# GAMES-UChile/mogptk

Hardware: AMD Instinct MI355X
Metric: log-marginal-likelihood+grad evals/sec, MOSM C=4 N=8192; 1/2/4/8 GPU (higher is better)
Workload: dtype f64

## Files before the change

include/mogp_hip.h:

```cpp
#ifndef MOGP_HIP_H
#define MOGP_HIP_H

#include <stdint.h>

#ifdef __cplusplus
extern "C" {
#endif

#define MOGP_OK            0
#define MOGP_EINVAL       -1
#define MOGP_EHIP         -2
#define MOGP_ENOTPD       -3
#define MOGP_ENONFINITE   -4
#define MOGP_ENODEVICE    -5

#define MOGP_TERM_WIDTH(D) (2 + 3 * (D))
#define MOGP_MOMENT_WIDTH(D) (2 + 3 * (D))

typedef struct mogp_ctx mogp_ctx;
typedef struct mogp_model mogp_model;

const char* mogp_version(void);
const char* mogp_last_error(void);
int  mogp_device_count(void);
// ... 91 lines not shown
int  mogp_stage_ms(mogp_model* m, double* ms, int64_t* gemm_launches, double* gemm_flops);

#define MOGP_SCHED_DATAFLOW            1
#define MOGP_SCHED_CHAIN_KERNEL        2
#define MOGP_SCHED_DATAFLOW_FELL_BACK  4
#define MOGP_SCHED_TIMEOUTS_SHIFT      8
#define MOGP_SCHED_CHAIN_FELL_BACK     8
int  mogp_model_schedule(mogp_model* m, int* flags);

int  mogp_model_flow_replay(mogp_model* m, int on);

int  mogp_model_flow_diag(mogp_model* m, unsigned* out8);

int  mogp_flow_plan(int nb, int64_t* out, int64_t cap, int64_t* count);
int  mogp_flow_plan_rhs(int nb, int rhs_nt, int64_t* out, int64_t cap, int64_t* count);
int  mogp_flow_trace(mogp_model* m, int64_t* out, int64_t cap, int64_t* count);

int  mogp_model_fetch(mogp_model* m, int which, double* out);

int  mogp_snelson_eval(mogp_model* m, int64_t M, const double* Z, const double* noise_var, double jitter, const double* kff_diag, int flags,
                       double* lml, double* mom_uu, double* mom_uf, double* gZ, double* trGA, double* hsum, double* jitter_abs, int64_t* info);
int  mogp_snelson_predict(mogp_model* m, int64_t M, const double* Z, const double* noise_var, double jitter, const double* kff_diag,
                          const double* kss_diag, int64_t S, const double* Xs, double* mu, double* var, int64_t* info);
int  mogp_snelson_eval_sharded(mogp_model* m, int64_t M, const double* Z, const double* noise_var, double jitter, const double* kff_diag,
                               int flags, double* lml, double* mom_uu, double* mom_uf, double* gZ, double* trGA, double* hsum,
                               double* jitter_abs, int64_t* info);
int  mogp_snelson_predict_sharded(mogp_model* m, int64_t M, const double* Z, const double* noise_var, double jitter, const double* kff_diag,
                                  const double* kss_diag, int64_t S, const double* Xs, double* mu, double* var, int64_t* info);

int  mogp_svgp_forward(mogp_model* m, int64_t M, const double* Z, const double* q_mu, const double* q_sqrt, double jitter,
// ... 25 lines not shown
```

mogptk_amd/_lib.py:

```python
import atexit
import ctypes
import os
import threading
import weakref
import numpy as np

_HERE = os.path.dirname(os.path.abspath(__file__))
LIB_PATH = os.environ.get("MOGP_LIB_PATH") or os.path.join(_HERE, "csrc", "libmogp_hip.so")

MOGP_OK, MOGP_EINVAL, MOGP_EHIP, MOGP_ENOTPD, MOGP_ENONFINITE, MOGP_ENODEVICE = 0, -1, -2, -3, -4, -5
MOGP_EVAL_GRAD = 1
COMM_ID_BYTES = 128
ALLGATHER_CB = ctypes.CFUNCTYPE(ctypes.c_int, ctypes.c_void_p, ctypes.c_void_p, ctypes.c_void_p, ctypes.c_int64)
ALLREDUCE_CB = ctypes.CFUNCTYPE(ctypes.c_int, ctypes.c_void_p, ctypes.c_void_p, ctypes.c_int64)
ST_GRAM, ST_POTRF, ST_TRTRI, ST_LAUUM, ST_SOLVE, ST_MOMENTS, ST_TOTAL, ST_GEMM_KERNEL, ST_GRAM_KERNEL, ST_MOMENT_KERNEL, ST_COUNT = range(11)

_lib = None
_lock = threading.RLock()
_ctx = {}
_live = weakref.WeakSet()

c_dp = ctypes.POINTER(ctypes.c_double)
c_i64p = ctypes.POINTER(ctypes.c_int64)
c_ip = ctypes.POINTER(ctypes.c_int)
# ... 56 lines not shown
    "mogp_shard_begin": (ctypes.c_int, [ctypes.c_void_p, c_dp, c_dp, ctypes.c_double, c_dp, ctypes.POINTER(ctypes.c_int)]),
    "mogp_shard_pack": (ctypes.c_int, [ctypes.c_void_p, ctypes.c_int, ctypes.POINTER(ctypes.c_void_p), ctypes.POINTER(ctypes.c_void_p), c_i64p]),
    "mogp_shard_unpack": (ctypes.c_int, [ctypes.c_void_p, ctypes.c_int]),
    "mogp_shard_block": (ctypes.c_int, [ctypes.c_void_p, ctypes.c_int]),
    "mogp_shard_alpha": (ctypes.c_int, [ctypes.c_void_p, ctypes.POINTER(ctypes.c_void_p), c_i64p]),
    "mogp_shard_finish": (ctypes.c_int, [ctypes.c_void_p, c_dp, c_dp, c_dp, c_i64p]),
    "mogp_dev_copy": (ctypes.c_int, [ctypes.c_void_p, ctypes.c_void_p, ctypes.c_int64, ctypes.c_int]),
    "mogp_set_profiling": (ctypes.c_int, [ctypes.c_void_p, ctypes.c_int]),
    "mogp_stage_ms": (ctypes.c_int, [ctypes.c_void_p, c_dp, c_i64p, c_dp]),
    "mogp_model_fetch": (ctypes.c_int, [ctypes.c_void_p, ctypes.c_int, c_dp]),
    "mogp_model_schedule": (ctypes.c_int, [ctypes.c_void_p, ctypes.POINTER(ctypes.c_int)]),
    "mogp_model_flow_replay": (ctypes.c_int, [ctypes.c_void_p, ctypes.c_int]),
    "mogp_model_flow_diag": (ctypes.c_int, [ctypes.c_void_p, ctypes.POINTER(ctypes.c_uint)]),
    "mogp_flow_plan": (ctypes.c_int, [ctypes.c_int, c_i64p, ctypes.c_int64, c_i64p]),
    "mogp_flow_plan_rhs": (ctypes.c_int, [ctypes.c_int, ctypes.c_int, c_i64p, ctypes.c_int64, ctypes.POINTER(ctypes.c_int64)]),
    "mogp_flow_trace": (ctypes.c_int, [ctypes.c_void_p, c_i64p, ctypes.c_int64, c_i64p]),
    "mogp_snelson_eval": (ctypes.c_int, [ctypes.c_void_p, ctypes.c_int64, c_dp, c_dp, ctypes.c_double, c_dp, ctypes.c_int,
                                         ctypes.POINTER(ctypes.c_double), c_dp, c_dp, c_dp, ctypes.POINTER(ctypes.c_double), c_dp,
                                         ctypes.POINTER(ctypes.c_double), c_i64p]),
    "mogp_snelson_predict": (ctypes.c_int, [ctypes.c_void_p, ctypes.c_int64, c_dp, c_dp, ctypes.c_double, c_dp, c_dp, ctypes.c_int64, c_dp,
                                            c_dp, c_dp, c_i64p]),
    "mogp_snelson_eval_sharded": (ctypes.c_int, [ctypes.c_void_p, ctypes.c_int64, c_dp, c_dp, ctypes.c_double, c_dp, ctypes.c_int,
                                         ctypes.POINTER(ctypes.c_double), c_dp, c_dp, c_dp, ctypes.POINTER(ctypes.c_double), c_dp,
                                         ctypes.POINTER(ctypes.c_double), c_i64p]),
    "mogp_snelson_predict_sharded": (ctypes.c_int, [ctypes.c_void_p, ctypes.c_int64, c_dp, c_dp, ctypes.c_double, c_dp, c_dp, ctypes.c_int64, c_dp,
                                            c_dp, c_dp, c_i64p]),
    "mogp_svgp_forward": (ctypes.c_int, [ctypes.c_void_p, ctypes.c_int64, c_dp, c_dp, c_dp, ctypes.c_double, c_dp, ctypes.c_int, ctypes.c_int64,
                                         c_dp, c_dp, c_dp, c_dp, ctypes.POINTER(ctypes.c_double), c_i64p]),
    "mogp_svgp_backward": (ctypes.c_int, [ctypes.c_void_p, c_dp, c_dp, c_dp, c_dp, c_dp, ctypes.POINTER(ctypes.c_double), c_dp, c_dp]),
    "mogp_svgp_backward_sharded": (ctypes.c_int, [ctypes.c_void_p, c_dp, c_dp, c_dp, c_dp, c_dp, ctypes.POINTER(ctypes.c_double), c_dp, c_dp]),
# ... 477 lines not shown
```

mogptk_amd/csrc/flow.hip:

```cpp
#include "mogp_model.h"
#include <unistd.h>
#include <chrono>
#include <set>

#include <cstdio>
#include <cstdlib>

namespace mogp {

typedef double d4_t __attribute__((ext_vector_type(4)));
typedef double d2_t __attribute__((ext_vector_type(2)));

#define FL_BK 16
#define FL_ROWK 18
#define FL_WTM 4
#define FL_WTN 2
#define FL_NWJ 4
#define FL_NWI 2
#define FL_NT 512
#define FL_COLK (MOGP_TILE + 16)
#define FL_OPER (MOGP_TILE * FL_ROWK)
#define FL_LDS_DOUBLES (2 * 2 * FL_OPER)
#define FL_LDS_BYTES (FL_LDS_DOUBLES * 8 + 16 + 3 * 64 * 4 + 16)
static_assert(MOGP_TILE * FL_ROWK == 16 * FL_COLK, "one LDS operand slot serves both layouts");

#define FL_LDS_BARRIER() asm volatile("s_waitcnt lgkmcnt(0)\n\ts_barrier" ::: "memory")

template <int AKM, int BKM, bool MARK = false>
__device__ __forceinline__ void flow_tile(const double* Ap, const double* Bp, double* Cp, const int64_t ld, const int kt, const bool fresh,
                                          const double alpha, double* gemm_lds, unsigned long long* tr, unsigned* prog, double* const* Cpp, const double* alphap) {
    constexpr int WTM = FL_WTM, WTN = FL_WTN, NWJ = FL_NWJ, NWI = FL_NWI, NT = FL_NT;
    constexpr int TMR = MOGP_TILE, TNC = MOGP_TILE, COLK_A = FL_COLK, COLK_B = FL_COLK, OPER_A = FL_OPER, OPER_B = FL_OPER;
    constexpr int EPT_A = TMR * FL_BK / NT, EPT_B = TNC * FL_BK / NT;
    constexpr int NQ_A = EPT_A / 2, NQ_B = EPT_B / 2, TPR_A = FL_BK / EPT_A, TPR_B = FL_BK / EPT_B, TPK = NT / FL_BK;
    int tl = threadIdx.x;
    asm volatile("" : "+v"(tl));
    const int ln = tl & 63, wv = tl >> 6, wi = wv / NWJ, wj = wv % NWJ;
    const int64_t a_g = AKM ? (int64_t)(tl / TPK) * ld + (tl % TPK) * EPT_A : (int64_t)(tl / TPR_A) * ld + (tl % TPR_A) * EPT_A;
    const int64_t b_g = BKM ? (int64_t)(tl / TPK) * ld + (tl % TPK) * EPT_B : (int64_t)(tl / TPR_B) * ld + (tl % TPR_B) * EPT_B;
    const int a_l = AKM ? (tl / TPK) * COLK_A + (tl % TPK) * EPT_A : (tl / TPR_A) * FL_ROWK + (tl % TPR_A) * EPT_A;
    const int b_l = BKM ? (tl / TPK) * COLK_B + (tl % TPK) * EPT_B : (tl / TPR_B) * FL_ROWK + (tl % TPR_B) * EPT_B;
    const int64_t a_step = AKM ? (int64_t)FL_BK * ld : FL_BK;
    const int64_t b_step = BKM ? (int64_t)FL_BK * ld : FL_BK;
    const int crow = wi * (TMR / NWI) + (ln >> 4), ccol = wj * (TNC / NWJ) + (ln & 15);
    const int fa = AKM ? (ln >> 4) * COLK_A + wi * (TMR / NWI) + (ln & 15) : (wi * (TMR / NWI) + (ln & 15)) * FL_ROWK + (ln >> 4);
    const int fb = BKM ? (ln >> 4) * COLK_B + wj * (TNC / NWJ) + (ln & 15) : (wj * (TNC / NWJ) + (ln & 15)) * FL_ROWK + (ln >> 4);
    constexpr int fa_m = AKM ? 16 : 16 * FL_ROWK, fa_k = AKM ? 4 * COLK_A : 4;
    constexpr int fb_n = BKM ? 16 : 16 * FL_ROWK, fb_k = BKM ? 4 * COLK_B : 4;

    d4_t acc[WTM][WTN];
    if (!fresh) {
#pragma unroll
        for (int m = 0; m < WTM; ++m)
#pragma unroll
            for (int n = 0; n < WTN; ++n)
#pragma unroll
                for (int r = 0; r < 4; ++r) acc[m][n][r] = alpha * Cp[(int64_t)(crow + m * 16 + 4 * r) * ld + ccol + n * 16];
    } else {
#pragma unroll
        for (int m = 0; m < WTM; ++m)
#pragma unroll
            for (int n = 0; n < WTN; ++n) acc[m][n] = (d4_t){0.0, 0.0, 0.0, 0.0};
    }
    d2_t ra[NQ_A], rb[NQ_B];
    auto load_block = [&](int kb) {
        const d2_t* pa = reinterpret_cast<const d2_t*>(Ap + a_g + (int64_t)kb * a_step);
        const d2_t* pb = reinterpret_cast<const d2_t*>(Bp + b_g + (int64_t)kb * b_step);
#pragma unroll
        for (int q = 0; q < NQ_A; ++q) ra[q] = pa[q];
#pragma unroll
        for (int q = 0; q < NQ_B; ++q) rb[q] = pb[q];
    };
// ... 1 lines not shown
        double* sa = gemm_lds + buf * (OPER_A + OPER_B);
        double* sb = sa + OPER_A;
#pragma unroll
        for (int q = 0; q < NQ_A; ++q) *reinterpret_cast<d2_t*>(sa + a_l + 2 * q) = ra[q];
#pragma unroll
        for (int q = 0; q < NQ_B; ++q) *reinterpret_cast<d2_t*>(sb + b_l + 2 * q) = rb[q];
    };
    auto read_frag = [&](double (&av)[WTM], double (&bv)[WTN], int buf, int k4) {
        const double* sa = gemm_lds + buf * (OPER_A + OPER_B);
        const double* sb = sa + OPER_A;
#pragma unroll
        for (int m = 0; m < WTM; ++m) av[m] = sa[fa + m * fa_m + k4 * fa_k];
#pragma unroll
        for (int n = 0; n < WTN; ++n) bv[n] = sb[fb + n * fb_n + k4 * fb_k];
    };
    auto mma = [&](const double (&av)[WTM], const double (&bv)[WTN]) {
#pragma unroll
        for (int m = 0; m < WTM; ++m)
#pragma unroll
            for (int n = 0; n < WTN; ++n)
                acc[m][n] = __builtin_amdgcn_mfma_f64_16x16x4f64(av[m], bv[n], acc[m][n], 0, 0, 0);
    };
#define FL_MARK(v) do { if constexpr (MARK) { if (prog && ln == 0) { const unsigned v__ = (v); prog[wv] = v__; \
        if (wv == 0) { const unsigned kb__ = v__ & 0xffffu, now__ = (unsigned)(wall_clock64() >> 4); \
            if (v__ == 0x10000u) prog[8] = now__; else if (v__ == 0x30000u) prog[13] = now__; else if (v__ == 0x40000u) prog[14] = now__; \
            else if ((v__ >> 16) == 2u && (kb__ & 7u) == 0u) prog[9 + (kb__ >> 3)] = now__; } } } } while (0)
    FL_MARK(0x10000u);
    load_block(0);
    write_block(0);
    load_block(min(1, kt - 1));
    FL_LDS_BARRIER();
    if constexpr (MARK) { if (tr) tr[2] = wall_clock64(); }
    {
        double a0[WTM], b0[WTN], a1[WTM], b1[WTN];
        read_frag(a0, b0, 0, 0);
        for (int kb = 0; kb < kt; ++kb) {
            const int buf = kb & 1;
            read_frag(a1, b1, buf, 1);
            __builtin_amdgcn_sched_barrier(0);
            mma(a0, b0);
            __builtin_amdgcn_sched_barrier(0);
            read_frag(a0, b0, buf, 2);
            __builtin_amdgcn_sched_barrier(0);
            mma(a1, b1);
            __builtin_amdgcn_sched_barrier(0);
            write_block(buf ^ 1);
            FL_MARK(0x20000u + (unsigned)kb);
            load_block(min(kb + 2, kt - 1));
            read_frag(a1, b1, buf, 3);
            __builtin_amdgcn_sched_barrier(0);
            mma(a0, b0);
            __builtin_amdgcn_sched_barrier(0);
            FL_LDS_BARRIER();
            read_frag(a0, b0, buf ^ 1, 0);
            __builtin_amdgcn_sched_barrier(0);
            mma(a1, b1);
            __builtin_amdgcn_sched_barrier(0);
        }
    }
    FL_MARK(0x30000u);
    if constexpr (MARK) { if (tr) tr[3] = wall_clock64(); }
    int t2 = threadIdx.x;
    asm volatile("" : "+v"(t2));
    const int ln2 = t2 & 63, wv2 = t2 >> 6;
    const int crow2 = (wv2 / NWJ) * (TMR / NWI) + (ln2 >> 4), ccol2 = (wv2 % NWJ) * (TNC / NWJ) + (ln2 & 15);
    double* Cq = *Cpp;
    const double alpha2 = *alphap;
#pragma unroll
    for (int m = 0; m < WTM; ++m)
#pragma unroll
        for (int n = 0; n < WTN; ++n)
#pragma unroll
            for (int r = 0; r < 4; ++r)
                __hip_atomic_store(Cq + (int64_t)(crow2 + m * 16 + 4 * r) * ld + ccol2 + n * 16, alpha2 * acc[m][n][r], __ATOMIC_RELAXED,
                                   __HIP_MEMORY_SCOPE_AGENT);
    FL_MARK(0x40000u);
#undef FL_MARK
}

struct FlowArgs {
    double* bA; double* bL; double* bWt; double* bWm; double* bB;
    int64_t ld;
    const FlowTask* tasks;
    const int* qmeta;
    unsigned* flags;
    int nq, ncas, base_heads, base_err;
    unsigned nap_max;
    unsigned nap_calm;
    int nhi;
    int claim_one;
    int refill;
    const double* vy; double* vz; double* vzz; double* vpart;
    int64_t npad;
    unsigned long long* info;
    int post_base;
    unsigned char* done;
    unsigned* post;
    unsigned* diag;
    unsigned long long* trace;
};

struct FlowHot {
    double* bA; double* bL; double* bWt; double* bWm; double* bB; int64_t ld;
    const FlowTask* tasks; const int* qmeta; unsigned* flags;
    int nq, ncas, base_heads, base_err;
    unsigned nap_max, nap_calm;
};

__device__ __forceinline__ void flow_zrow(const FlowArgs& g, const int i, double* lds) {
    int tid = threadIdx.x;
    asm volatile("" : "+v"(tid));
    const int lane = tid & 63, wave = tid >> 6;
    const int K = (i + 1) * MOGP_TILE;
    const double* Wr = g.bWm + (int64_t)(i * MOGP_TILE + wave * 16) * g.ld + 2 * lane;
    const double* yp = g.vy + 2 * lane;
    double zsq = 0.0;
    for (int r4 = 0; r4 < 16; r4 += 4) {
        const double* p0 = Wr + (int64_t)r4 * g.ld;
        d2_t a0 = (d2_t){0.0, 0.0}, a1 = a0, a2 = a0, a3 = a0;
#pragma unroll 2
        for (int k = 0; k < K; k += MOGP_TILE) {
// ... 213 lines not shown
                if (lane == 0) { po[0] = (unsigned)(res + 4); po[1] = idle; po[2] = 3u; po[5] = (unsigned)(wall_clock64() >> 4); }
            }
        }
        __syncthreads();
        const int ti = __builtin_amdgcn_readfirstlane(pick[0]);
        if (ti < 0) {
            if (ti == -3 && tid == 0) atomicMin(g.info, (unsigned long long)MOGP_INFO_CHAIN_TIMEOUT);
            break;
        }
        const FlowTask* tp = ha.tasks + ti;
        const int var = tp->var, kt = tp->kt;
        const int ab = tp->abuf, bb = tp->bbuf, cb = tp->cbuf;
        const double* Ab = ab == 0 ? ha.bA : ab == 1 ? ha.bL : ab == 2 ? ha.bWt : ab == 3 ? ha.bWm : ha.bB;
        const double* Bb = bb == 0 ? ha.bA : bb == 1 ? ha.bL : bb == 2 ? ha.bWt : bb == 3 ? ha.bWm : ha.bB;
        double* Cb = cb == 0 ? ha.bA : cb == 1 ? ha.bL : cb == 2 ? ha.bWt : cb == 3 ? ha.bWm : ha.bB;
        const double* Ap = Ab + ((int64_t)tp->ar * ha.ld + tp->ac) * MOGP_TILE;
        const double* Bp = Bb + ((int64_t)tp->br * ha.ld + tp->bc) * MOGP_TILE;
        double* Cp = Cb + ((int64_t)tp->cr * ha.ld + tp->cc) * MOGP_TILE;
        const bool fresh = (var & 4) != 0;
        const double alpha = (var & 8) ? -1.0 : 1.0;
        unsigned long long* tr = (MARK && g.trace && tid == 0) ? g.trace + FLOW_TRACE_W * (size_t)ti : nullptr;
        if (tr) { tr[0] = t_look; tr[1] = wall_clock64(); }
        unsigned* prog = (MARK && g.post) ? g.post + (size_t)(g.post_base + blockIdx.x) * FLOW_POST_W + 80 : nullptr;
        if (MARK && g.post && tid == 0) {
            unsigned* po = g.post + (size_t)(g.post_base + blockIdx.x) * FLOW_POST_W;
            po[2] = 2u; po[3] = (unsigned)ti; po[73] += 1u; po[76] = (unsigned)(wall_clock64() >> 4);
        }
        if (var & 32) {
            if (g.vy) {
                if (var & 1) flow_apart(g, tp->ar * MOGP_TILE, kt * MOGP_TILE, tp->br, tp->ac, gemm_lds);
                else flow_zrow(g, tp->ar, gemm_lds);
            }
        } else {
        if (var & 16) __builtin_amdgcn_s_setprio(2);
        if (tid == 0) { *ep_C = Cp; *ep_alpha = alpha; }
        switch (var & 3) {
            case 0: flow_tile<0, 0, MARK>(Ap, Bp, Cp, ha.ld, kt, fresh, alpha, gemm_lds, tr, prog, ep_C, ep_alpha); break;
            case 1: flow_tile<0, 1, MARK>(Ap, Bp, Cp, ha.ld, kt, fresh, alpha, gemm_lds, tr, prog, ep_C, ep_alpha); break;
            default: flow_tile<1, 1, MARK>(Ap, Bp, Cp, ha.ld, kt, fresh, alpha, gemm_lds, tr, prog, ep_C, ep_alpha); break;
        }
        if (var & 16) __builtin_amdgcn_s_setprio(0);
        }
        asm volatile("s_waitcnt vmcnt(0)" ::: "memory");
        __syncthreads();
        if (tid == 0) {
            const unsigned s0 = tp->sig[0], s1 = tp->sig[1];
            if (s0 != FLOW_NOSIG) __hip_atomic_fetch_add(ha.flags + s0, 1u, __ATOMIC_RELAXED, __HIP_MEMORY_SCOPE_AGENT);
            if (s1 != FLOW_NOSIG) __hip_atomic_fetch_add(ha.flags + s1, 1u, __ATOMIC_RELAXED, __HIP_MEMORY_SCOPE_AGENT);
            if (MARK && g.done) g.done[ti] = 1;
            if (MARK && g.post) g.post[(size_t)(g.post_base + blockIdx.x) * FLOW_POST_W + 77] = (unsigned)(wall_clock64() >> 4);
            if (tr) {
                tr[4] = wall_clock64();
                tr[5] = ((unsigned long long)(unsigned)pick[1] << 32) | ((unsigned long long)__builtin_amdgcn_s_getreg((3 << 11) | 20) << 16) | blockIdx.x;
            }
        }
    }
}


namespace {
enum { PH_INTO = 0, PH_CHAIN = 600, PH_T6 = 601, PH_PANEL = 602, PH_UPDATE = 603, PH_T9 = 604, PH_ZROW = 605, PH_APART = 606, PH_XS = 607, PH_TU = 608 };
enum { Q_LOOK2 = 0, Q_INVCRIT = 1, Q_SEMI = 2 };
enum { BUF_A = 0, BUF_L = 1, BUF_WT = 2, BUF_WM = 3, BUF_B = 4 };
}

void flow_build(int nb, int ob, FlowPlan& p, int rhs_nt, bool replay) {
    p = FlowPlan();
    p.nb = nb; p.ob = ob; p.rhs_nt = rhs_nt; p.replay = replay;
    const int no = (nb + ob - 1) / ob;
    p.nouter = no;
    const uint32_t base_S = 0, base_R = base_S + (uint32_t)nb * nb, base_DG = base_R + (uint32_t)nb * no, base_PN = base_DG + no,
                   base_CH = base_PN + (uint32_t)no * nb, base_WT = base_CH + no, base_WC = base_WT + (uint32_t)nb * nb,
                   base_WF = base_WC + (uint32_t)no * nb, base_KV = base_WF + (uint32_t)no * nb, base_WR = base_KV + (uint32_t)nb * nb,
                   base_ZR = base_WR + no, base_TS = base_ZR + no, base_TR = base_TS + (uint32_t)rhs_nt * nb, base_XN = base_TR + (uint32_t)rhs_nt * no,
                   base_end = base_XN + (uint32_t)no * rhs_nt;
    p.base_heads = (int)base_end; p.base_err = p.base_heads + FLOW_MAXQ; p.nflags = p.base_err + 1;
    auto S = [&](int i, int j) { return base_S + (uint32_t)i * nb + j; };
    auto R = [&](int i, int c) { return base_R + (uint32_t)i * no + c; };
// ... 19 lines not shown
    std::vector<std::vector<FlowTask>> into(no), trail(no);
    auto mk = [&](int b, int phase, int var, int kt) {
        FlowTask t{};
        t.var = (uint8_t)var; t.kt = (uint16_t)kt; t.ndep = 0; t.sig[0] = t.sig[1] = FLOW_NOSIG; t.key = (uint32_t)(b * FLOW_KEY_STEP + phase);
        return t;
    };
    auto dep = [&](FlowTask& t, uint32_t idx, unsigned need) {
        if (need == 0) return;
        t.dep[t.ndep] = idx; t.need[t.ndep] = (uint16_t)need; ++t.ndep;
    };
    auto opA = [](FlowTask& t, int buf, int r, int c) { t.abuf = (uint8_t)buf; t.ar = (uint16_t)r; t.ac = (uint16_t)c; };
    auto opB = [](FlowTask& t, int buf, int r, int c) { t.bbuf = (uint8_t)buf; t.br = (uint16_t)r; t.bc = (uint16_t)c; };
    auto opC = [](FlowTask& t, int buf, int r, int c) { t.cbuf = (uint8_t)buf; t.cr = (uint16_t)r; t.cc = (uint16_t)c; };
    const int KB = MOGP_TILE / FL_BK;
    double tiles_k = 0.0;

    auto crit_row = [&](int b, int i) { return !replay && i >= k1(b) && i < std::min(nb, k1(b) + ob); };
    auto pn_need = [&](int b, int i) { return (unsigned)((crit_row(b, i) ? 2 : 1) * nk(b)); };
    auto panel = [&](int b, int i, int c, bool prio) {
        FlowTask t = mk(b, PH_PANEL, 0 | 4 | (prio ? 16 : 0), KB * (c + 1));
        opA(t, BUF_A, i, k0(b)); opB(t, BUF_WM, k0(b) + c, k0(b)); opC(t, BUF_L, i, k0(b) + c);
        dep(t, CH(b), chain_wgs(b));
        dep(t, R(i, b), (unsigned)(nk(b) * b));
        t.sig[0] = PN(b, i);
        tiles_k += t.kt;
        return t;
    };
    auto update = [&](int b, int i, int j, bool prio) {
        FlowTask t = mk(b, PH_UPDATE, 0 | 8 | (prio ? 16 : 0), KB * nk(b));
        opA(t, BUF_L, i, k0(b)); opB(t, BUF_L, j, k0(b)); opC(t, BUF_A, i, j);
        dep(t, PN(b, i), pn_need(b, i));
        if (j != i) dep(t, PN(b, j), pn_need(b, j));
        dep(t, S(i, j), (unsigned)b);
        t.sig[0] = S(i, j);
        t.sig[1] = blk(i) == blk(j) ? DG(blk(j)) : R(i, blk(j));
        tiles_k += t.kt;
        return t;
    };
    auto t7 = [&](int b, int i, int c) {
        FlowTask t = mk(blk(i), PH_INTO + 2 * b, 1 | 4 | 8, KB * (nk(b) - c));
        opA(t, BUF_L, i, k0(b) + c); opB(t, BUF_WM, k0(b) + c, k0(b) + c); opC(t, BUF_WT, i, k0(b) + c);
        dep(t, PN(b, i), pn_need(b, i));
        t.sig[0] = WT(i, k0(b) + c); t.sig[1] = WC(blk(i), k0(b) + c);
        tiles_k += t.kt;
        return t;
    };
    auto t8 = [&](int b, int i, int j) {
        FlowTask t = mk(blk(i), PH_INTO + 2 * b + 1, 1 | 8, KB * nk(b));
        opA(t, BUF_L, i, k0(b)); opB(t, BUF_WM, k0(b), j); opC(t, BUF_WT, i, j);
        dep(t, PN(b, i), pn_need(b, i));
        dep(t, WF(b, j), (unsigned)nk(b));
        dep(t, WT(i, j), (unsigned)(b - blk(j)));
        t.sig[0] = WT(i, j); t.sig[1] = WC(blk(i), j);
        tiles_k += t.kt;
        return t;
    };
    auto t6 = [&](int b, int ti, int j) {
        FlowTask t = mk(b, PH_T6, 1 | 4, KB * (ti + 1));
        opA(t, BUF_WM, k0(b) + ti, k0(b)); opB(t, BUF_WT, k0(b), j); opC(t, BUF_WM, k0(b) + ti, j);
        dep(t, CH(b), chain_wgs(b));
        dep(t, WC(b, j), (unsigned)(nk(b) * (b - blk(j))));
        t.sig[0] = WF(b, j); t.sig[1] = WR(b);
        tiles_k += t.kt;
        return t;
    };
    static const bool t9_full = std::getenv("MOGP_FLOW_T9FULL") && std::atoi(std::getenv("MOGP_FLOW_T9FULL")) != 0;
    auto t9 = [&](int b, int i, int j) {
        const int r0 = (i >= k0(b) && !t9_full) ? i : k0(b);
        FlowTask t = mk(b, PH_T9, 2 | (i >= k0(b) ? 4 : 0), KB * (k1(b) - r0));
        opA(t, BUF_WM, r0, i); opB(t, BUF_WM, r0, j); opC(t, BUF_B, i, j);
        bool ch = false;
        if (i >= k0(b)) { dep(t, CH(b), chain_wgs(b)); ch = true; } else dep(t, WF(b, i), (unsigned)nk(b));
        if (j != i) { if (j >= k0(b)) { if (!ch) dep(t, CH(b), chain_wgs(b)); } else dep(t, WF(b, j), (unsigned)nk(b)); }
        dep(t, KV(i, j), (unsigned)(b - blk(i)));
        t.sig[0] = KV(i, j);
        tiles_k += t.kt;
        return t;
    };

    auto xs = [&](int b, int i, int c) {
        FlowTask t = mk(b, PH_XS, 0 | 4, KB * (c + 1));
        opA(t, BUF_WT, i, k0(b)); opB(t, BUF_WM, k0(b) + c, k0(b)); opC(t, BUF_B, i, k0(b) + c);
        dep(t, CH(b), chain_wgs(b));
        dep(t, TR(i, b), (unsigned)(nk(b) * b));
        t.sig[0] = XN(b, i);
        tiles_k += t.kt;
        return t;
    };
    auto tu = [&](int b, int i, int j) {
        FlowTask t = mk(b, PH_TU, 0 | 8, KB * nk(b));
        opA(t, BUF_B, i, k0(b)); opB(t, BUF_L, j, k0(b)); opC(t, BUF_WT, i, j);
        dep(t, XN(b, i), (unsigned)nk(b));
        dep(t, PN(b, j), pn_need(b, j));
        dep(t, TS(i, j), (unsigned)b);
        t.sig[0] = TS(i, j); t.sig[1] = TR(i, blk(j));
        tiles_k += t.kt;
        return t;
    };
    std::vector<FlowTask> rrest;

// ... 56 lines not shown
    if ((int)order.size() > FLOW_MAXQ) {
        std::vector<FlowTask> rest;
        std::vector<const std::vector<FlowTask>*> tail(order.begin() + (FLOW_MAXQ - 2), order.end() - 1);
        for (auto* v : tail) rest.insert(rest.end(), v->begin(), v->end());
        std::stable_sort(rest.begin(), rest.end(), [](const FlowTask& x, const FlowTask& y) { return x.key < y.key; });
        p.folded = rest;
        order.erase(order.begin() + (FLOW_MAXQ - 2), order.end() - 1);
        order.insert(order.end() - 1, &p.folded);
    }
    p.nq = (int)order.size();
    for (int qi = 0; qi < p.nq; ++qi) {
        p.qbase[qi] = (int)p.tasks.size(); p.qsize[qi] = (int)order[qi]->size();
        p.tasks.insert(p.tasks.end(), order[qi]->begin(), order[qi]->end());
    }
    p.flops = 2.0 * MOGP_TILE * MOGP_TILE * FL_BK * tiles_k;
}

__global__ void k_alpha_sum(const double* __restrict__ part, int64_t npad, int no, int ob, double* __restrict__ out) {
    const int64_t col = (int64_t)blockIdx.x * blockDim.x + threadIdx.x;
    if (col >= npad) return;
    double s = 0.0;
    for (int r = (int)(col / MOGP_TILE) / ob; r < no; ++r) s += part[(int64_t)r * npad + col];
    out[col] = s;
}
int launch_flow_alpha_sum(const Spd& w, double* alpha, hipStream_t st) {
    const FlowPlan& p = w.flow_cur ? *w.flow_cur : w.flow;
    hipLaunchKernelGGL(k_alpha_sum, dim3((unsigned)((w.Npad + 255) / 256)), dim3(256), 0, st, w.vec_part, w.Npad, p.nouter, p.ob, alpha);
    HIP_TRY(hipGetLastError());
    return 0;
}

bool flow_enabled(const mogp_model* m, const Spd& w) {
    const char* eo = std::getenv("MOGP_FLOW");
    const char* en = std::getenv("MOGP_FLOW_MIN");
    const int on = eo ? std::atoi(eo) : 1, nmin = en ? std::atoi(en) : 8;
    if (!on || (m->no_flow && m->n_fact < m->flow_retry_at) || !chain_enabled(m) || !m->ctx->st_priv) return false;
    if (m->kinv_sparse && &w == &m->k) return false;
    return w.nb >= nmin && w.nb <= 0xfff0;
}

int spd_potri_flow(mogp_model* m, Spd& w, const FlowRhs* rhs) {
    const int nb = w.nb, ob = 4;
    const int64_t ld = w.Npad;
    int rc;
    const auto host_t0 = std::chrono::steady_clock::now();
    hipStream_t crit = m->st, priv = m->st_priv, bulk = m->st2;
    if (w.Wm.n < (size_t)ld * ld) {
        if ((rc = w.Wm.ensure((size_t)ld * ld))) return rc;
        HIP_TRY(hipMemsetAsync(w.Wm.p, 0, (size_t)ld * ld * sizeof(double), crit));
    }
    if ((rc = w.Lm.ensure((size_t)ld * ld))) return rc;
    if (!rhs && (rc = w.Wt.ensure((size_t)ld * ld))) return rc;
    const bool replay = m->replay_flow && !rhs && &w == &m->k;
    FlowPlan& plan = rhs ? w.flow_rhs : replay ? w.flow_replay : w.flow;
    DevBuf<FlowTask>& d_tasks = rhs ? w.flow_tasks_rhs : replay ? w.flow_tasks_replay : w.flow_tasks;
    DevBuf<int>& d_qmeta = rhs ? w.flow_qmeta_rhs : replay ? w.flow_qmeta_replay : w.flow_qmeta;
    const int rhs_nt = rhs ? rhs->nt : 0;
    if (plan.nb != nb || plan.ob != ob || plan.rhs_nt != rhs_nt) {
        flow_build(nb, ob, plan, rhs_nt, replay);
// ... 89 lines not shown
        char* held = w.flow_args_h.data() + slot;
        char* fresh_ = w.flow_args_h.data() + 1024 + slot;
        std::memset(fresh_, 0, 512);
        std::memcpy(fresh_, &a, sizeof(a));
        if (std::memcmp(held, fresh_, 512) == 0) return 0;
        HIP_TRY(hipStreamSynchronize(st));
        HIP_TRY(dev_upload(w.flow_args.p + slot, fresh_, 512));
        std::memcpy(held, fresh_, 512);
        return 0;
    };
    if ((rc = upload(0, g, bulk))) return rc;
    const FlowArgs* d_g = reinterpret_cast<const FlowArgs*>(w.flow_args.p);
    FlowHot hot{};
    hot.bA = g.bA; hot.bL = g.bL; hot.bWt = g.bWt; hot.bWm = g.bWm; hot.bB = g.bB; hot.ld = g.ld; hot.tasks = g.tasks; hot.qmeta = g.qmeta; hot.flags = g.flags;
    hot.nq = g.nq; hot.ncas = g.ncas; hot.base_heads = g.base_heads; hot.base_err = g.base_err; hot.nap_max = g.nap_max; hot.nap_calm = g.nap_calm;
    if (dbg_kernel) hipLaunchKernelGGL(k_flow<true>, dim3(wg_per_cu * cus), dim3(FL_NT), FL_LDS_BYTES, bulk, d_g, hot);
    else hipLaunchKernelGGL(k_flow<false>, dim3(wg_per_cu * cus), dim3(FL_NT), FL_LDS_BYTES, bulk, d_g, hot);
    HIP_TRY(hipGetLastError());
    if (pe1) HIP_TRY(hipEventRecord(pe1, bulk));
    HIP_TRY(hipEventRecord(e_flow, bulk));
    m->gemm_launches += 1;
    m->gemm_flops += p.flops;

    unsigned* ferr = w.flow_flags.p + p.base_err;
    for (int kb = 0; kb < nouter && !replay; ++kb) {
        const int k0 = kb * ob, k1 = std::min(k0 + ob, nb), nk = k1 - k0, na = std::min(ob, nb - k1);
        const FlowPlan::Chain& pc = p.chain[kb];
        ChainFlow cf{};
        cf.done_flag = w.flow_flags.p + pc.done_idx; cf.write_through = 1;
        cf.trace = want_trace ? w.flow_trace.p + FLOW_TRACE_W * p.tasks.size() + 4 * (size_t)kb : nullptr;
        cf.diag = w.flow_diag.p;
        if ((rc = launch_chain(w.A.p, ld, k0, nk, w.invd.p, w.logdet.p, m->d_info.p, 0, w.Wm.p + (int64_t)k0 * MOGP_TILE * (ld + 1), ld,
                               w.chain_flags.p + (size_t)kb * MOGP_CHAIN_FLAGS, ferr, priv, &cf))) return rc;
        if (na <= 0) continue;
        GemmArgs t1{};
        t1.A = w.A.p + (int64_t)k1 * MOGP_TILE * ld + (int64_t)k0 * MOGP_TILE; t1.lda = ld; t1.a_kmajor = 0;
        t1.B = w.Wm.p + (int64_t)k0 * MOGP_TILE * (ld + 1); t1.ldb = ld; t1.b_kmajor = 0;
// ... 245 lines not shown
        std::fill(o, o + W, 0);
        o[0] = -3; o[1] = (int64_t)b * FLOW_KEY_STEP + PH_UPDATE; o[2] = b; o[3] = k0; o[4] = k1 - k0; o[5] = k1; o[6] = na; o[13] = c.t2_wval ? 1 : 0;
        o[14] = c.t2_widx; o[18] = c.t2_wval; o[22] = -1;
        o += W;
    }
    for (int q = 0; q < p.nq; ++q)
        for (int k = 0; k < p.qsize[q]; ++k, o += W) {
            const FlowTask& t = p.tasks[p.qbase[q] + k];
            o[0] = q; o[1] = t.key; o[2] = t.abuf; o[3] = t.ar; o[4] = t.ac; o[5] = t.bbuf; o[6] = t.br; o[7] = t.bc;
            o[8] = t.cbuf; o[9] = t.cr; o[10] = t.cc; o[11] = t.var; o[12] = t.kt; o[13] = t.ndep;
            for (int d = 0; d < 4; ++d) { o[14 + d] = d < t.ndep ? t.dep[d] : 0; o[18 + d] = d < t.ndep ? t.need[d] : 0; }
            o[22] = t.sig[0] == FLOW_NOSIG ? -1 : (int64_t)t.sig[0]; o[23] = t.sig[1] == FLOW_NOSIG ? -1 : (int64_t)t.sig[1];
        }
    return MOGP_OK;
}
```

mogptk_amd/csrc/mogp_internal.h:

```cpp
#pragma once
#include <hip/hip_runtime.h>
#include <stdint.h>
#include <atomic>
#include <string>
#include <vector>

#define MOGP_TILE 128
#define MOGP_GT 64
#define MOGP_TC 8
#define MOGP_MAXD 8

#define MOGP_KIND_GAUSS 0
#define MOGP_KIND_RQ 1
#define MOGP_KIND_MATERN12 2
#define MOGP_KIND_MATERN32 3
#define MOGP_KIND_MATERN52 4
#ifndef MOGP_KIND_PERIODIC
#define MOGP_KIND_PERIODIC 5
#endif
#ifndef MOGP_KIND_SINC
#define MOGP_KIND_SINC 6
#define MOGP_KIND_DOT 7
#define MOGP_DOT_DEGREE_MAX 8
#endif
// ... 196 lines not shown

#define FLOW_MAXQ 48
#define FLOW_NCAS 1
#define FLOW_TRACE_W 6
#define FLOW_POST_W 96
#define FLOW_KEY_STEP 1024
#define FLOW_NOSIG 0xffffffffu
struct FlowTask {
    uint16_t ar, ac, br, bc, cr, cc;
    uint8_t abuf, bbuf, cbuf, var;
    uint16_t kt, ndep;
    uint32_t dep[4];
    uint16_t need[4];
    uint32_t sig[2];
    uint32_t key;
    uint32_t pad[2];
};
static_assert(sizeof(FlowTask) == 64, "FlowTask layout");
enum { FLOW_DIAG_DEEP = 0, FLOW_DIAG_HEAD_STALE = 1, FLOW_DIAG_DEP_STALE = 2, FLOW_DIAG_WAIT_DEEP = 3, FLOW_DIAG_WAIT_STALE = 4, FLOW_DIAG_LAST = 5, FLOW_DIAG_WORDS = 8 };
struct FlowPlan {
    int nb = 0, ob = 0, nouter = 0, nq = 0, rhs_nt = 0;
    bool replay = false;
    std::vector<FlowTask> tasks;
    std::vector<FlowTask> folded;
    int qbase[FLOW_MAXQ] = {0}, qsize[FLOW_MAXQ] = {0};
    int nflags = 0, base_heads = 0, base_err = 0;
    struct Chain { uint32_t done_idx, expect; int t1_nwait; uint32_t t1_widx[4], t1_wval[4], t1_sig_base, t1_sig_per_row; uint32_t t2_widx, t2_wval; };
    std::vector<Chain> chain;
    double flops = 0.0;
};
void flow_build(int nb, int ob, FlowPlan& p, int rhs_nt = 0, bool replay = false);
int launch_pad_identity(double* A, int64_t ld, int64_t N, int64_t Npad, hipStream_t s);
int launch_trmv_lower(const double* W, int64_t ld, int64_t n, const double* y, double* z, double* zz_partial, hipStream_t s,
                      int row_mod = 0, int row_rem = 0);
int launch_trmv_lower_t(const double* W, int64_t ld, int64_t n, const double* z, double* a, hipStream_t s, int row_mod = 0, int row_rem = 0);
int launch_gemv_rows(const double* M, int64_t ld, int64_t rows, int64_t n, const double* v, double* out, hipStream_t s);
int launch_row_sqnorm_sub(const double* M, int64_t ld, int64_t rows, int64_t n, const double* base, double* out, hipStream_t s);
int launch_symv_lower(const double* A, int64_t ld, int64_t n, const double* y, double* out, double* scratch, double sign, hipStream_t s,
                      int row_mod = 0, int row_rem = 0);
int launch_copy2d(double* dst, int64_t ldd, const double* src, int64_t lds, int64_t rows, int64_t cols, double scale, hipStream_t s);
int launch_add_diag(double* A, int64_t ld, int64_t n, double val, hipStream_t s);
int launch_symmetrize(double* A, int64_t ld, int64_t n, hipStream_t s);
int launch_combine(double* out, const double* P, const double* Q, int64_t ld, int64_t n, double ca, double cp, double cq, hipStream_t s);
int launch_gemv_cols(const double* M, int64_t ld, int64_t rows, int64_t n, const double* v, double* out, double* scratch, hipStream_t s);
// ... 10 lines not shown
```

Before: 93.44.

## Skip MFMA sub-tiles that triangular and symmetric operands make zero or redundant

Tags each dataflow GEMM task with triangularity/symmetry flags (triangular operands on the last/first k-block, symmetric diagonal outputs) and predicates the f64 MFMA sub-tile updates and the C loads/stores with wave ballots, so work on known-zero or mirrored 16x16 blocks is skipped. The sub-tile-to-wave mapping is permuted (mirrored rows and columns) to balance the skipped work across waves. Operand base offsets are made wave-uniform via readfirstlane. An env knob selects the level and defaults to full skipping. This adds templated kernel variants, with more register pressure and code size, and per-iteration mask logic.

```diff
diff --git a/include/mogp_hip.h b/include/mogp_hip.h
--- a/include/mogp_hip.h
+++ b/include/mogp_hip.h
@@ -129,6 +129,7 @@
 
 int  mogp_flow_plan(int nb, int64_t* out, int64_t cap, int64_t* count);
 int  mogp_flow_plan_rhs(int nb, int rhs_nt, int64_t* out, int64_t cap, int64_t* count);
+int  mogp_flow_plan_tri(int nb, int rhs_nt, int64_t* out, int64_t cap, int64_t* count);
 int  mogp_flow_trace(mogp_model* m, int64_t* out, int64_t cap, int64_t* count);
 
 int  mogp_model_fetch(mogp_model* m, int which, double* out);
diff --git a/mogptk_amd/_lib.py b/mogptk_amd/_lib.py
--- a/mogptk_amd/_lib.py
+++ b/mogptk_amd/_lib.py
@@ -94,6 +94,7 @@
     "mogp_model_flow_diag": (ctypes.c_int, [ctypes.c_void_p, ctypes.POINTER(ctypes.c_uint)]),
     "mogp_flow_plan": (ctypes.c_int, [ctypes.c_int, c_i64p, ctypes.c_int64, c_i64p]),
     "mogp_flow_plan_rhs": (ctypes.c_int, [ctypes.c_int, ctypes.c_int, c_i64p, ctypes.c_int64, ctypes.POINTER(ctypes.c_int64)]),
+    "mogp_flow_plan_tri": (ctypes.c_int, [ctypes.c_int, ctypes.c_int, c_i64p, ctypes.c_int64, c_i64p]),
     "mogp_flow_trace": (ctypes.c_int, [ctypes.c_void_p, c_i64p, ctypes.c_int64, c_i64p]),
     "mogp_snelson_eval": (ctypes.c_int, [ctypes.c_void_p, ctypes.c_int64, c_dp, c_dp, ctypes.c_double, c_dp, ctypes.c_int,
                                          ctypes.POINTER(ctypes.c_double), c_dp, c_dp, c_dp, ctypes.POINTER(ctypes.c_double), c_dp,
diff --git a/mogptk_amd/csrc/flow.hip b/mogptk_amd/csrc/flow.hip
--- a/mogptk_amd/csrc/flow.hip
+++ b/mogptk_amd/csrc/flow.hip
@@ -26,36 +26,68 @@
 
 #define FL_LDS_BARRIER() asm volatile("s_waitcnt lgkmcnt(0)\n\ts_barrier" ::: "memory")
 
-template <int AKM, int BKM, bool MARK = false>
+__device__ __forceinline__ int fl_row_sub(const int slot) { const int wi = slot >> 2, m = slot & 3; return 4 * (m >> 1) + ((m & 1) ? 3 - wi : wi); }
+__device__ __forceinline__ int fl_col_sub(const int slot) { const int wj = slot >> 1; return (slot & 1) ? 7 - wj : wj; }
+
+template <int AKM, int BKM, bool MARK = false, bool TRI = false>
 __device__ __forceinline__ void flow_tile(const double* Ap, const double* Bp, double* Cp, const int64_t ld, const int kt, const bool fresh,
-                                          const double alpha, double* gemm_lds, unsigned long long* tr, unsigned* prog, double* const* Cpp, const double* alphap) {
+                                          const double alpha, double* gemm_lds, unsigned long long* tr, unsigned* prog, double* const* Cpp, const double* alphap,
+                                          const unsigned tri) {
     constexpr int WTM = FL_WTM, WTN = FL_WTN, NWJ = FL_NWJ, NWI = FL_NWI, NT = FL_NT;
+    static_assert(WTM == 4 && WTN == 2 && NWI == 2 && NWJ == 4 && MOGP_TILE == 128, "the sub-tile ownership and the predicate bits are written for 2 x 4 waves of 4 x 2 MFMA tiles");
     constexpr int TMR = MOGP_TILE, TNC = MOGP_TILE, COLK_A = FL_COLK, COLK_B = FL_COLK, OPER_A = FL_OPER, OPER_B = FL_OPER;
     constexpr int EPT_A = TMR * FL_BK / NT, EPT_B = TNC * FL_BK / NT;
     constexpr int NQ_A = EPT_A / 2, NQ_B = EPT_B / 2, TPR_A = FL_BK / EPT_A, TPR_B = FL_BK / EPT_B, TPK = NT / FL_BK;
     int tl = threadIdx.x;
     asm volatile("" : "+v"(tl));
     const int ln = tl & 63, wv = tl >> 6, wi = wv / NWJ, wj = wv % NWJ;
-    const int64_t a_g = AKM ? (int64_t)(tl / TPK) * ld + (tl % TPK) * EPT_A : (int64_t)(tl / TPR_A) * ld + (tl % TPR_A) * EPT_A;
-    const int64_t b_g = BKM ? (int64_t)(tl / TPK) * ld + (tl % TPK) * EPT_B : (int64_t)(tl / TPR_B) * ld + (tl % TPR_B) * EPT_B;
+    static_assert(EPT_A <= 16 && 16 % EPT_A == 0 && EPT_B <= 16 && 16 % EPT_B == 0, "a thread's share of a k-major block lies inside one sub-tile");
+    const int a_p = AKM ? (tl % TPK) * EPT_A : tl / TPR_A, b_p = BKM ? (tl % TPK) * EPT_B : tl / TPR_B;
+    const int a_x = 16 * fl_row_sub(a_p >> 4) + (a_p & 15), b_x = 16 * fl_col_sub(b_p >> 4) + (b_p & 15);
+    const int64_t a_g = AKM ? (int64_t)(tl / TPK) * ld + a_x : (int64_t)a_x * ld + (tl % TPR_A) * EPT_A;
+    const int64_t b_g = BKM ? (int64_t)(tl / TPK) * ld + b_x : (int64_t)b_x * ld + (tl % TPR_B) * EPT_B;
     const int a_l = AKM ? (tl / TPK) * COLK_A + (tl % TPK) * EPT_A : (tl / TPR_A) * FL_ROWK + (tl % TPR_A) * EPT_A;
     const int b_l = BKM ? (tl / TPK) * COLK_B + (tl % TPK) * EPT_B : (tl / TPR_B) * FL_ROWK + (tl % TPR_B) * EPT_B;
     const int64_t a_step = AKM ? (int64_t)FL_BK * ld : FL_BK;
     const int64_t b_step = BKM ? (int64_t)FL_BK * ld : FL_BK;
-    const int crow = wi * (TMR / NWI) + (ln >> 4), ccol = wj * (TNC / NWJ) + (ln & 15);
     const int fa = AKM ? (ln >> 4) * COLK_A + wi * (TMR / NWI) + (ln & 15) : (wi * (TMR / NWI) + (ln & 15)) * FL_ROWK + (ln >> 4);
     const int fb = BKM ? (ln >> 4) * COLK_B + wj * (TNC / NWJ) + (ln & 15) : (wj * (TNC / NWJ) + (ln & 15)) * FL_ROWK + (ln >> 4);
     constexpr int fa_m = AKM ? 16 : 16 * FL_ROWK, fa_k = AKM ? 4 * COLK_A : 4;
     constexpr int fb_n = BKM ? 16 : 16 * FL_ROWK, fb_k = BKM ? 4 * COLK_B : 4;
 
+    unsigned long long mk64 = ~0ull;
+    unsigned mall = 0xffu;
+    int ms = -8;
+    if constexpr (TRI) {
+        const int wvs = __builtin_amdgcn_readfirstlane(wv), wis = wvs / NWJ, wjs = wvs % NWJ;
+        const int pk = ln >> 3, pm = (ln >> 1) & 3, pn = ln & 1;
+        const int prs = 4 * (pm >> 1) + ((pm & 1) ? 3 - wis : wis), pcs = pn ? 7 - wjs : wjs;
+        const bool sym_on = !(tri & FLOW_TRI_SYM) || pcs <= prs;
+        bool on = sym_on;
+        if (tri & FLOW_TRI_B_LAST) on = on && pk <= pcs;
+        if (tri & FLOW_TRI_B_FIRST) on = on && pk >= pcs;
+        if (tri & FLOW_TRI_A_LAST) on = on && pk <= prs;
+        if (tri & FLOW_TRI_A_FIRST) on = on && pk >= prs;
+        mk64 = __builtin_amdgcn_ballot_w64(on);
+        mall = (unsigned)__builtin_amdgcn_ballot_w64(sym_on) & 0xffu;
+        if (tri & (FLOW_TRI_A_FIRST | FLOW_TRI_B_FIRST)) ms = 0;
+        else if (tri & (FLOW_TRI_A_LAST | FLOW_TRI_B_LAST)) ms = kt - 8;
+    }
+    auto maskof = [&](int kb) -> unsigned { return (kb >= ms && kb < ms + 8) ? (unsigned)(mk64 >> (8 * (kb - ms))) & 0xffu : mall; };
+
     d4_t acc[WTM][WTN];
     if (!fresh) {
+        const int crow_e = 16 * wi + (ln >> 4), crow_o = 16 * (3 - wi) + (ln >> 4), ccol_0 = 16 * wj + (ln & 15), ccol_1 = 16 * (7 - wj) + (ln & 15);
 #pragma unroll
         for (int m = 0; m < WTM; ++m)
 #pragma unroll
-            for (int n = 0; n < WTN; ++n)
-#pragma unroll
-                for (int r = 0; r < 4; ++r) acc[m][n][r] = alpha * Cp[(int64_t)(crow + m * 16 + 4 * r) * ld + ccol + n * 16];
+            for (int n = 0; n < WTN; ++n) {
+                if ((mall >> (2 * m + n)) & 1u) {
+#pragma unroll
+                    for (int r = 0; r < 4; ++r)
+                        acc[m][n][r] = alpha * Cp[(int64_t)(((m & 1) ? crow_o : crow_e) + 64 * (m >> 1) + 4 * r) * ld + (n ? ccol_1 : ccol_0)];
+                } else acc[m][n] = (d4_t){0.0, 0.0, 0.0, 0.0};
+            }
     } else {
 #pragma unroll
         for (int m = 0; m < WTM; ++m)
@@ -87,12 +119,12 @@
 #pragma unroll
         for (int n = 0; n < WTN; ++n) bv[n] = sb[fb + n * fb_n + k4 * fb_k];
     };
-    auto mma = [&](const double (&av)[WTM], const double (&bv)[WTN]) {
+    auto mma = [&](const double (&av)[WTM], const double (&bv)[WTN], const unsigned mk) {
 #pragma unroll
         for (int m = 0; m < WTM; ++m)
 #pragma unroll
             for (int n = 0; n < WTN; ++n)
-                acc[m][n] = __builtin_amdgcn_mfma_f64_16x16x4f64(av[m], bv[n], acc[m][n], 0, 0, 0);
+                if (!TRI || (mk & (1u << (2 * m + n)))) acc[m][n] = __builtin_amdgcn_mfma_f64_16x16x4f64(av[m], bv[n], acc[m][n], 0, 0, 0);
     };
 #define FL_MARK(v) do { if constexpr (MARK) { if (prog && ln == 0) { const unsigned v__ = (v); prog[wv] = v__; \
         if (wv == 0) { const unsigned kb__ = v__ & 0xffffu, now__ = (unsigned)(wall_clock64() >> 4); \
@@ -109,25 +141,26 @@
         read_frag(a0, b0, 0, 0);
         for (int kb = 0; kb < kt; ++kb) {
             const int buf = kb & 1;
+            const unsigned mk = TRI ? maskof(kb) : 0xffu;
             read_frag(a1, b1, buf, 1);
             __builtin_amdgcn_sched_barrier(0);
-            mma(a0, b0);
+            mma(a0, b0, mk);
             __builtin_amdgcn_sched_barrier(0);
             read_frag(a0, b0, buf, 2);
             __builtin_amdgcn_sched_barrier(0);
-            mma(a1, b1);
+            mma(a1, b1, mk);
             __builtin_amdgcn_sched_barrier(0);
             write_block(buf ^ 1);
             FL_MARK(0x20000u + (unsigned)kb);
             load_block(min(kb + 2, kt - 1));
             read_frag(a1, b1, buf, 3);
             __builtin_amdgcn_sched_barrier(0);
-            mma(a0, b0);
+            mma(a0, b0, mk);
             __builtin_amdgcn_sched_barrier(0);
             FL_LDS_BARRIER();
             read_frag(a0, b0, buf ^ 1, 0);
             __builtin_amdgcn_sched_barrier(0);
-            mma(a1, b1);
+            mma(a1, b1, mk);
             __builtin_amdgcn_sched_barrier(0);
         }
     }
@@ -135,20 +168,27 @@
     if constexpr (MARK) { if (tr) tr[3] = wall_clock64(); }
     int t2 = threadIdx.x;
     asm volatile("" : "+v"(t2));
-    const int ln2 = t2 & 63, wv2 = t2 >> 6;
-    const int crow2 = (wv2 / NWJ) * (TMR / NWI) + (ln2 >> 4), ccol2 = (wv2 % NWJ) * (TNC / NWJ) + (ln2 & 15);
+    const int ln2 = t2 & 63, wv2 = t2 >> 6, wi2 = wv2 / NWJ, wj2 = wv2 % NWJ;
+    const int crow_e2 = 16 * wi2 + (ln2 >> 4), crow_o2 = 16 * (3 - wi2) + (ln2 >> 4), ccol_02 = 16 * wj2 + (ln2 & 15), ccol_12 = 16 * (7 - wj2) + (ln2 & 15);
     double* Cq = *Cpp;
     const double alpha2 = *alphap;
 #pragma unroll
     for (int m = 0; m < WTM; ++m)
 #pragma unroll
         for (int n = 0; n < WTN; ++n)
-#pragma unroll
-            for (int r = 0; r < 4; ++r)
-                __hip_atomic_store(Cq + (int64_t)(crow2 + m * 16 + 4 * r) * ld + ccol2 + n * 16, alpha2 * acc[m][n][r], __ATOMIC_RELAXED,
-                                   __HIP_MEMORY_SCOPE_AGENT);
+            if ((mall >> (2 * m + n)) & 1u) {
+#pragma unroll
+                for (int r = 0; r < 4; ++r)
+                    __hip_atomic_store(Cq + (int64_t)(((m & 1) ? crow_o2 : crow_e2) + 64 * (m >> 1) + 4 * r) * ld + (n ? ccol_12 : ccol_02),
+                                       alpha2 * acc[m][n][r], __ATOMIC_RELAXED, __HIP_MEMORY_SCOPE_AGENT);
+            }
     FL_MARK(0x40000u);
 #undef FL_MARK
+}
+
+__device__ __forceinline__ int64_t fl_uniform(const int64_t v) {
+    const unsigned lo = __builtin_amdgcn_readfirstlane((unsigned)v), hi = __builtin_amdgcn_readfirstlane((unsigned)((unsigned long long)v >> 32));
+    return (int64_t)(((unsigned long long)hi << 32) | lo);
 }
 
 struct FlowArgs {
@@ -178,6 +218,7 @@
     const FlowTask* tasks; const int* qmeta; unsigned* flags;
     int nq, ncas, base_heads, base_err;
     unsigned nap_max, nap_calm;
+    unsigned tri_mask;
 };
 
 __device__ __forceinline__ void flow_zrow(const FlowArgs& g, const int i, double* lds) {
@@ -421,8 +462,8 @@
         const double* Ab = ab == 0 ? ha.bA : ab == 1 ? ha.bL : ab == 2 ? ha.bWt : ab == 3 ? ha.bWm : ha.bB;
         const double* Bb = bb == 0 ? ha.bA : bb == 1 ? ha.bL : bb == 2 ? ha.bWt : bb == 3 ? ha.bWm : ha.bB;
         double* Cb = cb == 0 ? ha.bA : cb == 1 ? ha.bL : cb == 2 ? ha.bWt : cb == 3 ? ha.bWm : ha.bB;
-        const double* Ap = Ab + ((int64_t)tp->ar * ha.ld + tp->ac) * MOGP_TILE;
-        const double* Bp = Bb + ((int64_t)tp->br * ha.ld + tp->bc) * MOGP_TILE;
+        const double* Ap = Ab + fl_uniform(((int64_t)tp->ar * ha.ld + tp->ac) * MOGP_TILE);
+        const double* Bp = Bb + fl_uniform(((int64_t)tp->br * ha.ld + tp->bc) * MOGP_TILE);
         double* Cp = Cb + ((int64_t)tp->cr * ha.ld + tp->cc) * MOGP_TILE;
         const bool fresh = (var & 4) != 0;
         const double alpha = (var & 8) ? -1.0 : 1.0;
@@ -441,10 +482,14 @@
         } else {
         if (var & 16) __builtin_amdgcn_s_setprio(2);
         if (tid == 0) { *ep_C = Cp; *ep_alpha = alpha; }
-        switch (var & 3) {
-            case 0: flow_tile<0, 0, MARK>(Ap, Bp, Cp, ha.ld, kt, fresh, alpha, gemm_lds, tr, prog, ep_C, ep_alpha); break;
-            case 1: flow_tile<0, 1, MARK>(Ap, Bp, Cp, ha.ld, kt, fresh, alpha, gemm_lds, tr, prog, ep_C, ep_alpha); break;
-            default: flow_tile<1, 1, MARK>(Ap, Bp, Cp, ha.ld, kt, fresh, alpha, gemm_lds, tr, prog, ep_C, ep_alpha); break;
+        const unsigned tri = tp->tri & ha.tri_mask;
+        switch ((var & 3) | (tri ? 4 : 0)) {
+            case 0: flow_tile<0, 0, MARK>(Ap, Bp, Cp, ha.ld, kt, fresh, alpha, gemm_lds, tr, prog, ep_C, ep_alpha, 0u); break;
+            case 1: flow_tile<0, 1, MARK>(Ap, Bp, Cp, ha.ld, kt, fresh, alpha, gemm_lds, tr, prog, ep_C, ep_alpha, 0u); break;
+            case 2: case 3: flow_tile<1, 1, MARK>(Ap, Bp, Cp, ha.ld, kt, fresh, alpha, gemm_lds, tr, prog, ep_C, ep_alpha, 0u); break;
+            case 4: flow_tile<0, 0, MARK, true>(Ap, Bp, Cp, ha.ld, kt, fresh, alpha, gemm_lds, tr, prog, ep_C, ep_alpha, tri); break;
+            case 5: flow_tile<0, 1, MARK, true>(Ap, Bp, Cp, ha.ld, kt, fresh, alpha, gemm_lds, tr, prog, ep_C, ep_alpha, tri); break;
+            default: flow_tile<1, 1, MARK, true>(Ap, Bp, Cp, ha.ld, kt, fresh, alpha, gemm_lds, tr, prog, ep_C, ep_alpha, tri); break;
         }
         if (var & 16) __builtin_amdgcn_s_setprio(0);
         }
@@ -469,6 +514,23 @@
 enum { PH_INTO = 0, PH_CHAIN = 600, PH_T6 = 601, PH_PANEL = 602, PH_UPDATE = 603, PH_T9 = 604, PH_ZROW = 605, PH_APART = 606, PH_XS = 607, PH_TU = 608 };
 enum { Q_LOOK2 = 0, Q_INVCRIT = 1, Q_SEMI = 2 };
 enum { BUF_A = 0, BUF_L = 1, BUF_WT = 2, BUF_WM = 3, BUF_B = 4 };
+long long tri_omitted(unsigned tri, int kt) {
+    if (!tri) return 0;
+    const bool sym = (tri & FLOW_TRI_SYM) != 0;
+    long long marked = 0;
+    for (int kb = 0; kb < 8; ++kb)
+        for (int rs = 0; rs < 8; ++rs)
+            for (int cs = 0; cs < 8; ++cs) {
+                bool on = !sym || cs <= rs;
+                if (tri & FLOW_TRI_B_LAST) on = on && kb <= cs;
+                if (tri & FLOW_TRI_B_FIRST) on = on && kb >= cs;
+                if (tri & FLOW_TRI_A_LAST) on = on && kb <= rs;
+                if (tri & FLOW_TRI_A_FIRST) on = on && kb >= rs;
+                marked += on ? 0 : 1;
+            }
+    const long long per_kb = sym ? 28 : 0;
+    return (tri & FLOW_TRI_OPERANDS) ? marked + per_kb * (kt - 8) : per_kb * kt;
+}
 }
 
 void flow_build(int nb, int ob, FlowPlan& p, int rhs_nt, bool replay) {
@@ -518,6 +580,12 @@
     auto opC = [](FlowTask& t, int buf, int r, int c) { t.cbuf = (uint8_t)buf; t.cr = (uint16_t)r; t.cc = (uint16_t)c; };
     const int KB = MOGP_TILE / FL_BK;
     double tiles_k = 0.0;
+    double omitted[3] = {0.0, 0.0, 0.0};
+    auto mark = [&](FlowTask& t, unsigned tri) {
+        t.tri = tri;
+        omitted[1] += (double)tri_omitted(tri & FLOW_TRI_OPERANDS, t.kt);
+        omitted[2] += (double)tri_omitted(tri, t.kt);
+    };
 
     auto crit_row = [&](int b, int i) { return !replay && i >= k1(b) && i < std::min(nb, k1(b) + ob); };
     auto pn_need = [&](int b, int i) { return (unsigned)((crit_row(b, i) ? 2 : 1) * nk(b)); };
@@ -527,6 +595,7 @@
         dep(t, CH(b), chain_wgs(b));
         dep(t, R(i, b), (unsigned)(nk(b) * b));
         t.sig[0] = PN(b, i);
+        mark(t, FLOW_TRI_B_LAST);
         tiles_k += t.kt;
         return t;
     };
@@ -538,6 +607,7 @@
         dep(t, S(i, j), (unsigned)b);
         t.sig[0] = S(i, j);
         t.sig[1] = blk(i) == blk(j) ? DG(blk(j)) : R(i, blk(j));
+        if (i == j) mark(t, FLOW_TRI_SYM);
         tiles_k += t.kt;
         return t;
     };
@@ -546,6 +616,7 @@
         opA(t, BUF_L, i, k0(b) + c); opB(t, BUF_WM, k0(b) + c, k0(b) + c); opC(t, BUF_WT, i, k0(b) + c);
         dep(t, PN(b, i), pn_need(b, i));
         t.sig[0] = WT(i, k0(b) + c); t.sig[1] = WC(blk(i), k0(b) + c);
+        mark(t, FLOW_TRI_B_FIRST);
         tiles_k += t.kt;
         return t;
     };
@@ -565,6 +636,7 @@
         dep(t, CH(b), chain_wgs(b));
         dep(t, WC(b, j), (unsigned)(nk(b) * (b - blk(j))));
         t.sig[0] = WF(b, j); t.sig[1] = WR(b);
+        mark(t, FLOW_TRI_A_LAST);
         tiles_k += t.kt;
         return t;
     };
@@ -578,6 +650,7 @@
         if (j != i) { if (j >= k0(b)) { if (!ch) dep(t, CH(b), chain_wgs(b)); } else dep(t, WF(b, j), (unsigned)nk(b)); }
         dep(t, KV(i, j), (unsigned)(b - blk(i)));
         t.sig[0] = KV(i, j);
+        mark(t, (r0 == i ? (unsigned)FLOW_TRI_A_FIRST | (j == i ? (unsigned)FLOW_TRI_B_FIRST : 0u) : 0u) | (j == i ? (unsigned)FLOW_TRI_SYM : 0u));
         tiles_k += t.kt;
         return t;
     };
@@ -588,6 +661,7 @@
         dep(t, CH(b), chain_wgs(b));
         dep(t, TR(i, b), (unsigned)(nk(b) * b));
         t.sig[0] = XN(b, i);
+        mark(t, FLOW_TRI_B_LAST);
         tiles_k += t.kt;
         return t;
     };
@@ -674,6 +748,7 @@
         p.tasks.insert(p.tasks.end(), order[qi]->begin(), order[qi]->end());
     }
     p.flops = 2.0 * MOGP_TILE * MOGP_TILE * FL_BK * tiles_k;
+    for (int l = 0; l < 3; ++l) p.flops_tri[l] = p.flops - 2.0 * 16 * 16 * 16 * omitted[l];
 }
 
 __global__ void k_alpha_sum(const double* __restrict__ part, int64_t npad, int no, int ob, double* __restrict__ out) {
@@ -703,6 +778,8 @@
     const int nb = w.nb, ob = 4;
     const int64_t ld = w.Npad;
     int rc;
+    const char* etri = std::getenv("MOGP_FLOW_TRI");
+    const int tri_level = etri ? std::min(2, std::max(0, std::atoi(etri))) : FLOW_TRI_DEFAULT;
     const auto host_t0 = std::chrono::steady_clock::now();
     hipStream_t crit = m->st, priv = m->st_priv, bulk = m->st2;
     if (w.Wm.n < (size_t)ld * ld) {
@@ -822,13 +899,14 @@
     FlowHot hot{};
     hot.bA = g.bA; hot.bL = g.bL; hot.bWt = g.bWt; hot.bWm = g.bWm; hot.bB = g.bB; hot.ld = g.ld; hot.tasks = g.tasks; hot.qmeta = g.qmeta; hot.flags = g.flags;
     hot.nq = g.nq; hot.ncas = g.ncas; hot.base_heads = g.base_heads; hot.base_err = g.base_err; hot.nap_max = g.nap_max; hot.nap_calm = g.nap_calm;
+    hot.tri_mask = tri_level >= 2 ? (unsigned)FLOW_TRI_ALL : tri_level == 1 ? (unsigned)FLOW_TRI_OPERANDS : 0u;
     if (dbg_kernel) hipLaunchKernelGGL(k_flow<true>, dim3(wg_per_cu * cus), dim3(FL_NT), FL_LDS_BYTES, bulk, d_g, hot);
     else hipLaunchKernelGGL(k_flow<false>, dim3(wg_per_cu * cus), dim3(FL_NT), FL_LDS_BYTES, bulk, d_g, hot);
     HIP_TRY(hipGetLastError());
     if (pe1) HIP_TRY(hipEventRecord(pe1, bulk));
     HIP_TRY(hipEventRecord(e_flow, bulk));
     m->gemm_launches += 1;
-    m->gemm_flops += p.flops;
+    m->gemm_flops += p.flops_tri[tri_level];
 
     unsigned* ferr = w.flow_flags.p + p.base_err;
     for (int kb = 0; kb < nouter && !replay; ++kb) {
@@ -1104,3 +1182,14 @@
         }
     return MOGP_OK;
 }
+extern "C" int mogp_flow_plan_tri(int nb, int rhs_nt, int64_t* out, int64_t cap, int64_t* count) {
+    if (nb <= 0 || nb > 4096 || rhs_nt < 0 || rhs_nt > 4096 || !count) return fail(MOGP_EINVAL, "mogp_flow_plan_tri: bad argument");
+    FlowPlan p;
+    flow_build(nb, 4, p, rhs_nt);
+    *count = (int64_t)p.tasks.size();
+    if (!out) return MOGP_OK;
+    if (cap < *count) return fail(MOGP_EINVAL, "mogp_flow_plan_tri: the output holds fewer than count numbers");
+    for (int q = 0; q < p.nq; ++q)
+        for (int k = 0; k < p.qsize[q]; ++k) *out++ = (int64_t)p.tasks[p.qbase[q] + k].tri;
+    return MOGP_OK;
+}
diff --git a/mogptk_amd/csrc/mogp_internal.h b/mogptk_amd/csrc/mogp_internal.h
--- a/mogptk_amd/csrc/mogp_internal.h
+++ b/mogptk_amd/csrc/mogp_internal.h
@@ -234,9 +234,13 @@
     uint16_t need[4];
     uint32_t sig[2];
     uint32_t key;
-    uint32_t pad[2];
+    uint32_t tri;
+    uint32_t pad;
 };
 static_assert(sizeof(FlowTask) == 64, "FlowTask layout");
+enum { FLOW_TRI_B_LAST = 1, FLOW_TRI_B_FIRST = 2, FLOW_TRI_A_LAST = 4, FLOW_TRI_A_FIRST = 8, FLOW_TRI_SYM = 16,
+       FLOW_TRI_OPERANDS = 15, FLOW_TRI_ALL = 31 };
+#define FLOW_TRI_DEFAULT 2
 enum { FLOW_DIAG_DEEP = 0, FLOW_DIAG_HEAD_STALE = 1, FLOW_DIAG_DEP_STALE = 2, FLOW_DIAG_WAIT_DEEP = 3, FLOW_DIAG_WAIT_STALE = 4, FLOW_DIAG_LAST = 5, FLOW_DIAG_WORDS = 8 };
 struct FlowPlan {
     int nb = 0, ob = 0, nouter = 0, nq = 0, rhs_nt = 0;
@@ -248,6 +252,7 @@
     struct Chain { uint32_t done_idx, expect; int t1_nwait; uint32_t t1_widx[4], t1_wval[4], t1_sig_base, t1_sig_per_row; uint32_t t2_widx, t2_wval; };
     std::vector<Chain> chain;
     double flops = 0.0;
+    double flops_tri[3] = {0.0, 0.0, 0.0};
 };
 void flow_build(int nb, int ob, FlowPlan& p, int rhs_nt = 0, bool replay = false);
 int launch_pad_identity(double* A, int64_t ld, int64_t N, int64_t Npad, hipStream_t s);
```

Result: no change. 93.87, median of 2 (+0.5%).
